# mmbell/Scythe.jl

Hardware: AMD Instinct MI355X
Metric: model steps/sec, RLZ 512x256x64 shallow-water (higher is better)
Workload: dtype f64; 1 GPU; RLZ 513x256x64 (rings x azimuth x levels), 6 vars, 7 derivative slots, Oneway_ShallowWater_HeightResolvedBL, uniform ring table kmax<=127, b_zDim 43; num_cells=171, tiles=1, exchange=none, exchange_impl=none, device_busy_before_warmup=500 steps of the timed model, nan=False

## Files before the change

### include/scythe_hip.h

```cpp
#ifndef SCYTHE_HIP_H
#define SCYTHE_HIP_H

#include <stddef.h>
#include <stdint.h>

#ifdef __cplusplus
extern "C" {
#endif

#define SX_ABI_VERSION 2

enum { SX_GEOM_R = 0, SX_GEOM_RZ = 1, SX_GEOM_RL = 2, SX_GEOM_RLZ = 3 };

enum { SX_BC_R0 = 0, SX_BC_R1T0 = 1, SX_BC_R1T1 = 2, SX_BC_R1T2 = 3, SX_BC_R2T10 = 4, SX_BC_R2T20 = 5, SX_BC_R3 = 6,
       SX_BC_PERIODIC = 7 };

enum {
    SX_EQ_LINEAR_ADVECTION_1D = 0,
    SX_EQ_LINEAR_ADVECTION_RZ = 1,
    SX_EQ_LINEAR_ADVECTION_RL = 2,
    SX_EQ_LINEAR_ADVECTION_RLZ = 3,
    SX_EQ_ONEWAY_SW_SLAB = 4,
    SX_EQ_TWOWAY_SW_SLAB = 5,
    SX_EQ_ONEWAY_SW_HRBL = 6,
// ... 61 lines not shown
int sx_abi_version(void);
int sx_equation_set_id(const char *name);
int sx_get_dims(const sx_handle *h, sx_dims *out);
int sx_set_stream(sx_handle *h, void *hip_stream);
int sx_synchronize(sx_handle *h);

int sx_get_gridpoints(const sx_handle *h, double *out);
int sx_calc_tile_sizes(const sx_grid_desc *patch, int32_t n_tiles, double *out);

int sx_cheb_column_ops(double zmin, double zmax, int32_t zDim, int32_t b_zDim, int32_t bcb, int32_t bct, double *z,
                       double *rec, double *dz, double *dzz, double *integ);

int sx_spline_solve_check(int32_t num_cells, double xmin, double xmax, double l_q, int32_t bcl, int32_t bcr, const double *b,
                          double *a_pcr, double *a_chol, int32_t *levels);

enum { SX_PLAN_FORWARD = 0, SX_PLAN_ZINV = 1, SX_PLAN_PCR = 2 };
int sx_launch_plan(int32_t kind, const int32_t *in, int32_t *out, char *kernel, int32_t kernel_cap);

int sx_set_physical_values(sx_handle *h, const double *values);
int sx_get_physical(sx_handle *h, double *out);
int sx_get_var_np1(sx_handle *h, double *out);
int sx_get_tile_spectral(sx_handle *h, double *out);
int sx_set_patch_spectral_b(sx_handle *h, const double *shared);
int sx_get_patch_spectral_a(sx_handle *h, double *out);
int sx_set_patch_spectral_a(sx_handle *h, const double *a);

int sx_index_map_sizes(const sx_handle *h, int64_t *n_owned, int64_t *n_halo);
int sx_index_maps(const sx_handle *h, int64_t *patch_owned, int64_t *tile_owned, int64_t *patch_halo, int64_t *tile_halo);

int sx_state_size(const sx_handle *h, int64_t *n_doubles);
int sx_get_state(sx_handle *h, double *out);
// ... 51 lines not shown
```

### scythe.jl_amd/csrc/sx_api.cpp

```cpp
#include "sx_internal.hpp"
#include <algorithm>
#include <array>
#include <cmath>
#include <cstdlib>
#include <cstring>
#include <map>
#include <type_traits>

namespace sx {

static thread_local std::string g_err;
static thread_local bool g_err_set = false;

void set_error(const std::string &msg) {
    if (!g_err_set) g_err = msg;
    g_err_set = true;
}
void clear_error() { g_err_set = false; }
static int status() { return g_err_set ? 1 : 0; }
int error_status() { return status(); }

#define HIPOK(x)                                                                          \
    do {                                                                                  \
        hipError_t e_ = (x);                                                              \
// ... 626 lines not shown
                    j.mat_off = ((int64_t)v * 3 + sz) * h->nz * h->Zb;
                    jf.push_back(j);
                    const int need = sz == 0 ? horiz : sz == 1 ? z : zz;
                    if (eq[v] & need) je.push_back(j);
                }
                ColJob f;
                f.in_off = (int64_t)v * h->nz * h->K2;
                f.out_off = (int64_t)v * h->Zb * h->K2;
                f.mat_off = 0;
                jz.push_back(f);
            }
            h->njobs_zinv_full = (int)jf.size();
            h->njobs_zinv_eq = (int)je.size();
            if (!upload(h, &h->d_jobs_zinv_full, jf) || !upload(h, &h->d_jobs_zinv_eq, je) || !upload(h, &h->d_jobs_zf, jz)) FAIL();
        }
    }
    {
        std::vector<int64_t> ao(h->b_rDim), neg(h->b_rDim, -1);
        for (int m = 0; m < h->b_rDim; m++) ao[m] = (int64_t)m * h->C;
        if (hipMemcpy(h->d_aoff, ao.data(), sizeof(int64_t) * ao.size(), hipMemcpyHostToDevice) != hipSuccess ||
            hipMemcpy(h->d_neg1, neg.data(), sizeof(int64_t) * neg.size(), hipMemcpyHostToDevice) != hipSuccess) {
            set_error("hipMemcpy H2D failed");
            FAIL();
        }
    }
    h->v_lo = 0; h->v_cnt = h->V;
    h->defer_diag = h->sw.defer_diag && h->eq == SX_EQ_ONEWAY_SW_HRBL && h->V == 6 && h->ncells == h->nc && mfma_shape(h, true) &&
                    h->sw.sbw_mfma;
    if (sx_bind_patch_b(h, nullptr, nullptr)) FAIL();
    *out = h;
// ... 7 lines not shown
#ifdef SX_PHASES
    phases_dump();
    fft_phases_dump();
    sbw_phases_dump();
    dft_phases_dump();
#endif
    graphs_release(h);
    if (h->graph_stream) hipStreamDestroy(h->graph_stream);
    comm_release(h);
    iface_release(h);
    pcr_release(h);
    for (auto &p : h->pending) { hipEventDestroy(p.a); hipEventDestroy(p.b); }
    for (auto e : h->event_pool) hipEventDestroy(e);
    if (h->ev_fork) hipEventDestroy(h->ev_fork);
    if (h->ev_join) hipEventDestroy(h->ev_join);
    if (h->stream2) hipStreamDestroy(h->stream2);
    for (void *p : h->allocs) hipFree(p);
    delete h;
    return 0;
}

int sx_cheb_column_ops(double zmin, double zmax, int32_t zDim, int32_t b_zDim, int32_t bcb, int32_t bct, double *z,
                       double *rec, double *dz, double *dzz, double *integ) {
    clear_error();
    if (zDim < 2 || !(zmax > zmin)) { set_error("sx_cheb_column_ops: need zDim >= 2 and zmax > zmin"); return 1; }
    const int Zb = b_zDim > 0 ? std::min(b_zDim, zDim) : std::min(zDim, (2 * zDim - 1) / 3 + 1);
    ChebOps o;
    std::string err;
    if (!build_cheb_ops(zmin, zmax, zDim, Zb, bcb, bct, o, err)) { set_error(err); return 1; }
    const size_t n2 = (size_t)zDim * zDim;
// ... 14 lines not shown
    std::string err;
    const int nb = num_cells + 3;
    if (!build_spline_class(num_cells, (xmax - xmin) / num_cells, l_q > 0 ? l_q : 2.0, bcl, bcr, sc, err) || !build_pcr_tables(sc, nb, t, err)) {
        set_error(err);
        return 1;
    }
    if (a_pcr) pcr_apply_host(t, nb, b, a_pcr);
    if (a_chol) cholesky_apply_host(sc, nb, b, a_chol);
    if (levels) *levels = t.levels;
    return 0;
}

int sx_launch_plan(int32_t kind, const int32_t *in, int32_t *out, char *kernel, int32_t kernel_cap) {
    clear_error();
    if (!in || !out) { set_error("sx_launch_plan: null argument"); return 1; }
    if (kind != SX_PLAN_FORWARD && kind != SX_PLAN_ZINV && kind != SX_PLAN_PCR) { set_error("sx_launch_plan: unknown kind " + std::to_string(kind)); return 1; }
    const int first = kind == SX_PLAN_PCR ? 0 : 1, last = kind == SX_PLAN_FORWARD ? 6 : kind == SX_PLAN_ZINV ? 3 : 4;
    for (int i = first; i < last; i++)
        if (in[i] < 1) { set_error("sx_launch_plan: dimensions must be positive"); return 1; }
    const Switches sw = read_switches();
    std::string name;
    if (kind == SX_PLAN_FORWARD) {
        const SbPlan p = plan_sb(in[0], in[1], in[2], in[3], in[4], in[5], in[6], sw);
        name = kernel_name(p.kernel);
        const int32_t o[6] = {p.threads, p.bw, p.groups, p.nseg, p.cps, p.segs};
        std::copy(o, o + 6, out);
    } else if (kind == SX_PLAN_ZINV) {
        const ZinvPlan p = plan_zinv(in[0], in[1], in[2], in[3], sw);
        name = kernel_name(p);
        out[0] = p.CT; out[1] = p.grid_x;
// ... 237 lines not shown
}

}

namespace sx {
void flush_diag(sx_handle *h) {
    if (!h->diag_dirty) return;
    h->diag_dirty = false;
    h->v_lo = h->V - 1; h->v_cnt = 1;
    launch_fl_forward(h);
    launch_sb(h);
    launch_solve(h);
    h->v_lo = 0; h->v_cnt = h->V;
}

static void step_launches(sx_handle *h, int t, bool solve) {
    launch_zinv(h, false);
    launch_inverse_and_physics(h, t);
    if (h->defer_diag) { h->v_cnt = h->V - 1; h->diag_dirty = true; }
    launch_fl_forward(h);
    launch_sb(h);
    if (solve) launch_solve(h);
    h->v_cnt = h->V;
}
}

extern "C" {

int sx_spectral_transform(sx_handle *h) {
    clear_error();
    if (!h) { set_error("null handle"); return 1; }
    h->diag_dirty = false;
    launch_fl_forward(h);
    launch_sb(h);
    return status();
}

// ... 343 lines not shown
```

### scythe.jl_amd/csrc/sx_fft.hip

```cpp
#include "sx_internal.hpp"
#include <cstdlib>
#include <cstdio>
#include <vector>

namespace sx {

template <int LOGL, int HL = 0> struct FftCfg {
    static constexpr int FZC = 16, FNP = FZC / 2, LOGZ = 4, SKEW = (LOGL <= 8) ? 2 : 0;
    static constexpr int L4 = (1 << LOGL) / 4;
    static constexpr int LPT = (L4 > 64 ? 64 : L4) >> HL;
    static constexpr int NB = L4 / LPT;
    static constexpr int NK = 2 * NB;
};

#ifdef SX_PHASES
__device__ long long *g_fft_dbg = nullptr;
#define FFT_STAMP(i) do { if (NODE && threadIdx.x == 0 && g_fft_dbg) g_fft_dbg[((int64_t)(blockIdx.z * gridDim.y + blockIdx.y) * gridDim.x + blockIdx.x) * 8 + (i)] = (long long)__builtin_readcyclecounter(); } while (0)
#else
#define FFT_STAMP(i) do { } while (0)
#endif

__device__ __forceinline__ double2 cmul(double2 a, double2 b) { return make_double2(a.x * b.x - a.y * b.y, a.x * b.y + a.y * b.x); }
__device__ __forceinline__ double2 cadd(double2 a, double2 b) { return make_double2(a.x + b.x, a.y + b.y); }
__device__ __forceinline__ double2 csub(double2 a, double2 b) { return make_double2(a.x - b.x, a.y - b.y); }
// ... 558 lines not shown
}

static int fft_fzc(int) { return 16; }
static size_t fft_lds(int L, int sets = 1, bool reg = false) { return sizeof(double2) * ((size_t)sets * (fft_fzc(L) / 2) * (L + (reg ? L / 16 + 2 : L <= 256 ? 2 : 0)) + (reg ? (L == 512 ? 448 : 192) : 0)); }
static int fft_threads(int L, int hl = 0) { return std::max(64, (fft_fzc(L) / 2) * (std::min(L / 4, 64) >> hl)); }

struct InvTarget {
    double *out;
    const double *phi;
    const int *kmax;
    const int64_t *pstart, *phoff;
    int n_units, n_phi;
    int64_t N;
    int node_mode;
    int unit0 = 0;
};

template <int LOGL>
static void launch_inv(sx_handle *h, const int *d_mask, const InvTarget &tg, const double *az, int64_t azrow) {
    const int L = 1 << LOGL;
    dim3 g((h->nz + fft_fzc(L) - 1) / fft_fzc(L), tg.n_units, h->V);
#define INV_LAUNCH_V(NODE, ST, AT, HL, SETS)                                                                                         \
    do {                                                                                                                             \
        if (fft_lds(L, SETS) > 65536)                                                                                                \
            HIPCHK(hipFuncSetAttribute(reinterpret_cast<const void *>(k_rl_inverse_fft<LOGL, 1, NODE, ST, AT, HL, SETS>),           \
                                        hipFuncAttributeMaxDynamicSharedMemorySize, (int)fft_lds(L, SETS)));                        \
        hipLaunchKernelGGL((k_rl_inverse_fft<LOGL, 1, NODE, ST, AT, HL, SETS>), g, dim3(fft_threads(L, HL)), fft_lds(L, SETS), h->stream, \
                           reinterpret_cast<const AT *>(az), planes_of<ST>(tg.out, h->V, tg.N), tg.phi, tg.kmax, tg.pstart,          \
                           h->d_tw, tg.phoff, h->d_ph, d_mask, h->V, h->nz, h->nsz, h->K2, tg.n_phi, tg.N, azrow, h->slot[0],        \
                           h->slot[1], h->slot[2], h->slot[3], h->slot[4], h->slot[5], h->slot[6], nullptr, (int64_t)0, nullptr, 0,  \
                           tg.unit0);                                                                                                \
    } while (0)
#define INV_LAUNCH_REG(NODE, ST, AT)                                                                                                 \
    do {                                                                                                                             \
        constexpr int RS = 2;                                                                                                        \
        if (fft_lds(L, RS, true) > 65536)                                                                                            \
// ... 41 lines not shown
}

template <int LOGL>
static void launch_fwd(sx_handle *h, dim3 g) {
    const int L = 1 << LOGL;
    if (h->sp32)
        hipLaunchKernelGGL((k_fl_forward_fft<LOGL, float>), g, dim3(fft_threads(L)), fft_lds(L), h->stream, h->d_np1 + (int64_t)h->v_lo * h->N,
                           reinterpret_cast<float *>(h->d_Fl) + (int64_t)h->v_lo * h->nz * h->K2,
                           h->d_kmax, h->d_pstart, h->d_tw, h->d_phoff, h->d_ph, h->V, h->nz, h->K2, h->N);
    else
        hipLaunchKernelGGL((k_fl_forward_fft<LOGL, double>), g, dim3(fft_threads(L)), fft_lds(L), h->stream, h->d_np1 + (int64_t)h->v_lo * h->N,
                           h->d_Fl + (int64_t)h->v_lo * h->nz * h->K2, h->d_kmax,
                           h->d_pstart, h->d_tw, h->d_phoff, h->d_ph, h->V, h->nz, h->K2, h->N);
}

void launch_rl_inverse_fft(sx_handle *h, const int *d_mask, int n_rings) {
    const int id = timer_id(h, "k_rl_inverse");
    timer_begin(h, id);
    InvTarget tg{h->d_phys, h->d_phi, h->d_kmax, h->d_pstart, h->d_phoff, n_rings < 0 ? h->nrings : n_rings, h->nrings, h->N, 0};
    launch_inv_any(h, d_mask, tg);
    timer_end(h);
}

#ifdef SX_PHASES
static long long *g_fft_buf = nullptr;
static int64_t g_fft_n = 0;
void fft_phases_dump() {
    const char *path = getenv("SX_FFT_PHASES_OUT");
    if (!path || !g_fft_buf) return;
    std::vector<long long> hst((size_t)g_fft_n * 8);
    hipDeviceSynchronize();
    hipMemcpy(hst.data(), g_fft_buf, sizeof(long long) * hst.size(), hipMemcpyDeviceToHost);
    FILE *f = fopen(path, "wb");
    if (f) { fwrite(hst.data(), sizeof(long long), hst.size(), f); fclose(f); }
}
#endif

void launch_node_fft(sx_handle *h) {
    const int id = timer_id(h, "k_node_fft");
    timer_begin(h, id);
#ifdef SX_PHASES
    if (!g_fft_buf) {
        g_fft_n = (int64_t)((h->nz + fft_fzc(h->uniform_L) - 1) / fft_fzc(h->uniform_L)) * h->V * h->nbt;
        hipMalloc(&g_fft_buf, sizeof(long long) * g_fft_n * 8);
        hipMemset(g_fft_buf, 0, sizeof(long long) * g_fft_n * 8);
        hipMemcpyToSymbol(HIP_SYMBOL(g_fft_dbg), &g_fft_buf, sizeof(g_fft_buf));
    }
#endif
    const int j0 = h->R_in / MUBAR;
    InvTarget tg{h->d_G, h->d_nphi, h->d_nkmax, h->d_npstart, h->d_nphoff, h->nbt - j0, h->nbt, h->NG, 1, j0};
    launch_inv_any(h, h->d_mask_node, tg);
    timer_end(h);
}

void launch_fl_forward_fft(sx_handle *h) {
    const int id = timer_id(h, "k_fl_forward");
    timer_begin(h, id);
    const int fzc = fft_fzc(h->uniform_L);
    dim3 g((h->nz + fzc - 1) / fzc, h->v_cnt, h->nrings);
    switch (ilog2(h->uniform_L)) {
        case 4: launch_fwd<4>(h, g); break;
        case 5: launch_fwd<5>(h, g); break;
        case 6: launch_fwd<6>(h, g); break;
        case 7: launch_fwd<7>(h, g); break;
        case 8: launch_fwd<8>(h, g); break;
        default: launch_fwd<9>(h, g); break;
// ... 7 lines not shown
```

### scythe.jl_amd/csrc/sx_internal.hpp

```cpp
#pragma once
#include <hip/hip_runtime.h>
#include <cmath>
#include <cstdint>
#include <string>
#include <utility>
#include <vector>
#include "scythe_hip.h"

#define HIPCHK(x)                                                                                   \
    do {                                                                                            \
        hipError_t e_ = (x);                                                                        \
        if (e_ != hipSuccess) ::sx::set_error(std::string(#x) + ": " + hipGetErrorString(e_) + " (" __FILE__ ":" + std::to_string(__LINE__) + ")"); \
    } while (0)

namespace sx {

void set_error(const std::string &msg);

constexpr int DFT_KMAX_SINGLE = 319;
constexpr int MUBAR = 3;

struct SplineClass {
    int bcl = 0, bcr = 0;
    int nfree = 0, periodic = 0, rl = 0, rr = 0;
// ... 112 lines not shown
    SbKernel kernel = SbKernel::refused;
    int threads = 0, bw = 0;
    int groups = 0, nseg = 0, cps = 0, segs = 0;
};
enum class ZinvKernel { none , colmat, mfma_2_1, mfma_4_1, mfma_4_2, mfma_8_1, mfma_8_2, mfma_8_4 };
struct ZinvPlan {
    ZinvKernel kernel = ZinvKernel::none;
    bool f32 = false;
    int CT = 1, grid_x = 0;
};
struct PcrPlan { int R = 1, logR = 0, threads = 64; };
constexpr int PCR_IPT = 4;
SbPlan plan_sb(int geometry, int nz, int Zb, int K2, int v_cnt, int ncells, int sp32, const Switches &sw);
ZinvPlan plan_zinv(int geometry, int nz, int K2, int sp32, const Switches &sw);
PcrPlan plan_pcr(int nblk_max, int b_rDim, int K2, int ngroups, const Switches &sw);
std::string kernel_name(SbKernel k);
std::string kernel_name(const ZinvPlan &p);

struct Timer {
    const char *name;
    double ms = 0.0;
    int64_t calls = 0;
};

struct PendingEvent {
    int timer;
    hipEvent_t a, b;
};

}
// ... 15 lines not shown
    double ts = 0;
    int eq = SX_EQ_NONE, semi = 0, w_index = 0, xi_index = 0, col_var = 0;
    double par[SX_NPARAMS] = {};
    int rot = 0;
    hipStream_t stream = nullptr;
    double *d_A = nullptr, *d_Bfull = nullptr, *d_Btile = nullptr, *d_Btile_own = nullptr;
    const double *d_Bsrc = nullptr;
    int64_t *d_rowoff = nullptr, *d_aoff = nullptr, *d_neg1 = nullptr;
    int a2a_n = 0, a2a_me = 0, a2a_g0 = 0, a2a_g1 = 0;
    std::vector<int64_t> a2a_colstart;
    std::vector<int> a2a_cell0, a2a_ncells;
    int *d_a2a_owner = nullptr;
    int64_t *d_a2a_soff = nullptr, *d_a2a_cw = nullptr, *d_a2a_cs = nullptr, *d_a2a_offA = nullptr, *d_a2a_offB = nullptr;
    hipStream_t stream2 = nullptr;
    hipEvent_t ev_fork = nullptr, ev_join = nullptr;
    int *d_dft_items[3] = {nullptr, nullptr, nullptr};
    int n_dft_items[3] = {0, 0, 0};
    int n_dft_big[3] = {0, 0, 0};
    int dft_lcap_small = 0, dft_kcap_small = 0;
    int plain_steps = 0;
    hipGraphExec_t graph_exec[3] = {nullptr, nullptr, nullptr};
    hipStream_t graph_stream = nullptr;
    int *d_rlq_items[2] = {nullptr, nullptr};
    int n_rlq_items[2] = {0, 0};
    int defer_diag = 0, v_lo = 0, v_cnt = 0;
    bool diag_dirty = false;
    std::vector<int> hmask_full, hmask_eq;
    bool in_advance = false;
    bool L_all_mult4 = false;
    sx::CellConsts cell_consts = {};
// ... 33 lines not shown
    sx::ColJob *d_jobs_zinv_full = nullptr, *d_jobs_zinv_eq = nullptr, *d_jobs_zf = nullptr;
    int njobs_zinv_full = 0, njobs_zinv_eq = 0, last_zinv_jobs = 0, last_zinv_rows = 0;
    int ncls = 0;
    size_t dev_bytes = 0;
    std::vector<void *> allocs;
    int timers_on = 0;
    bool timer_skip = false;
    std::string timer_only;
    std::vector<sx::Timer> timers;
    std::vector<sx::PendingEvent> pending;
    std::vector<hipEvent_t> event_pool;
};

namespace sx {
inline dim3 grid1(int64_t n, int bs) { return dim3((unsigned)((n + bs - 1) / bs)); }
void launch_zinv(sx_handle *h, bool full);
void launch_rl_inverse(sx_handle *h, bool full);
bool fft_path_ok(const sx_handle *h);
inline bool mfma_levels(int nz) { return nz == 32 || nz == 64 || nz == 128; }
inline bool mfma_shape(const sx_handle *h, bool zb_bound = false) {
    return fft_path_ok(h) && h->has_z && mfma_levels(h->nz) && (!zb_bound || (h->nz <= 64 ? h->Zb <= 64 : h->Zb <= 96));
}
bool fft_fused_zinv(const sx_handle *h);
bool dft_mfma_ok(const sx_handle *h);
void launch_rl_inverse_dft(sx_handle *h, const int *d_mask);
void launch_fl_forward_dft(sx_handle *h);
void launch_rl_inverse_fft(sx_handle *h, const int *d_mask, int n_rings = -1);
void launch_node_fft(sx_handle *h);
void launch_fl_forward_fft(sx_handle *h);
void launch_physics(sx_handle *h, int t);
void launch_inverse_and_physics(sx_handle *h, int t);
void launch_copy_slot0(sx_handle *h);
void launch_fl_forward(sx_handle *h);
void launch_sb(sx_handle *h);
void launch_solve(sx_handle *h);
void launch_solve_a2a(sx_handle *h, const double *recv, double *send);
void launch_a2a_pack(sx_handle *h, double *buf, int unpack);
void launch_halo_add(sx_handle *h, const double *recv);
void launch_nan_check(sx_handle *h);
void launch_max_abs(sx_handle *h, unsigned long long *d_out);
int timer_id(sx_handle *h, const char *name);
void timer_begin(sx_handle *h, int id);
void timer_end(sx_handle *h);
void timers_flush(sx_handle *h);
void clear_error();
int error_status();
void comm_release(sx_handle *h);
void flush_diag(sx_handle *h);
void graphs_release(sx_handle *h);
void iface_release(sx_handle *h);
// ... 17 lines not shown
```

### scythe.jl_amd/csrc/sx_kernels.hip

```cpp
#include "sx_internal.hpp"
#include <cmath>

namespace sx {

constexpr int ZC = 16;

__global__ void __launch_bounds__(256)
k_colmat(const double *__restrict__ in, double *__restrict__ out, const double *__restrict__ mats,
         const ColJob *__restrict__ jobs, int n_in, int n_out, int K2, int64_t in_row, int64_t out_row, int row0) {
    extern __shared__ double As[];
    const int lane = threadIdx.x;
    const int g = __builtin_amdgcn_readfirstlane(threadIdx.y);
    const int blk = blockIdx.x * 64 + lane;
    const ColJob job = jobs[blockIdx.y];
    const double *src = in + (int64_t)(row0 + blockIdx.z) * in_row + job.in_off;
    double *dst = out + (int64_t)blockIdx.z * out_row + job.out_off;
    const double *M = mats + job.mat_off;
    const bool ok = blk < K2;
    for (int i = g; i < n_in; i += 4) As[i * 64 + lane] = ok ? src[(int64_t)i * K2 + blk] : 0.0;
    __syncthreads();
    for (int o0 = g * 4; o0 < n_out; o0 += 16) {
        const double *m0 = M + (int64_t)o0 * n_in;
        const double *m1 = M + (int64_t)min(o0 + 1, n_out - 1) * n_in;
        const double *m2 = M + (int64_t)min(o0 + 2, n_out - 1) * n_in;
// ... 735 lines not shown

#ifdef SX_PHASES
static long long *g_sbw_buf = nullptr;
static int64_t g_sbw_n = 0;
void sbw_phases_dump() {
    const char *path = getenv("SX_SBW_PHASES_OUT");
    if (!path || !g_sbw_buf) return;
    std::vector<long long> hst((size_t)g_sbw_n * 8);
    hipDeviceSynchronize();
    hipMemcpy(hst.data(), g_sbw_buf, sizeof(long long) * hst.size(), hipMemcpyDeviceToHost);
    FILE *f = fopen(path, "wb");
    if (f) { fwrite(hst.data(), sizeof(long long), hst.size(), f); fclose(f); }
}
#endif

void launch_zinv(sx_handle *h, bool full) {
    if (!h->has_z || rz_fused(h)) return;
    const int id = timer_id(h, "k_zinv");
    timer_begin(h, id);
    const int njobs = full ? h->njobs_zinv_full : h->njobs_zinv_eq;
    h->last_zinv_jobs = njobs;
    if (njobs > 0) {
        const int rows = (!full && h->node_mode && fft_fused_zinv(h)) ? (h->R_in > 0 ? std::min(h->nbt, h->R_in / MUBAR + 3) : 0) : h->nbt;
        h->last_zinv_rows = rows;
        if (rows == 0) { timer_end(h); return; }
        const ZinvPlan p = plan_zinv(h->geom, h->nz, h->K2, h->sp32, h->sw);
        dim3 g(p.grid_x, njobs, rows);
        const ColJob *jobs = full ? h->d_jobs_zinv_full : h->d_jobs_zinv_eq;
        const int64_t azrow = (int64_t)h->V * 3 * h->nz * h->K2;
#define ZINV_T(MT, OT, CT) hipLaunchKernelGGL((k_colmat_mfma<MT, OT, CT>), g, dim3(256), 0, h->stream, h->d_A, reinterpret_cast<OT *>(h->d_Az), h->d_MzT, jobs, h->Zb, h->K2, h->C, azrow, h->cell0)
#define ZINV(MT, CT) if (p.f32) ZINV_T(MT, float, CT); else ZINV_T(MT, double, CT); break
        switch (p.kernel) {
        case ZinvKernel::mfma_2_1: ZINV(2, 1);
        case ZinvKernel::mfma_4_1: ZINV(4, 1);
        case ZinvKernel::mfma_4_2: ZINV(4, 2);
        case ZinvKernel::mfma_8_1: ZINV(8, 1);
        case ZinvKernel::mfma_8_2: ZINV(8, 2);
        case ZinvKernel::mfma_8_4: ZINV(8, 4);
        case ZinvKernel::colmat:
            hipLaunchKernelGGL(k_colmat, g, dim3(64, 4), sizeof(double) * 64 * h->Zb, h->stream, h->d_A, h->d_Az, h->d_Mz, jobs,
                               h->Zb, h->nz, h->K2, h->C, azrow, h->cell0);
            break;
        case ZinvKernel::none: break;
// ... 46 lines not shown
    const int id = timer_id(h, "k_fl_forward");
    timer_begin(h, id);
    const int xstride = h->L_max | 1;
    const size_t lds = sizeof(double) * ZC * xstride;
    if (lds > 64 * 1024) {
        set_error("azimuthal forward transform: rings of " + std::to_string(h->L_max) + " points are outside every transform path (power-of-two ring tables up to 512 points, ring lengths that are multiples of 4 up to 5120 points, any length up to 511 points)");
        return;
    }
    dim3 g((h->nz + ZC - 1) / ZC, h->V, h->nrings);
    hipLaunchKernelGGL(k_fl_forward, g, dim3(256), lds, h->stream, h->d_np1, h->d_Fl, h->d_L, h->d_kmax, h->d_pstart,
                       h->d_twoff, h->d_tw, h->d_phoff, h->d_ph, h->V, h->nz, h->K2, h->N, h->has_l, xstride);
    HIPCHK(hipGetLastError());
    timer_end(h);
}

void launch_sb(sx_handle *h) {
    const SbPlan p = plan_sb(h->geom, h->nz, h->Zb, h->K2, h->v_cnt, h->ncells, h->sp32, h->sw);
    if (p.kernel == SbKernel::rz_forward) { launch_rz_forward(h); return; }
    if (p.kernel == SbKernel::refused) { set_error("launch_sb: fp32 ring spectra (storage_f32 = 2) need the matrix-core sliding-window kernel"); return; }
    const int id = timer_id(h, h->has_z ? "k_sbz" : "k_sb");
    timer_begin(h, id);
    if (p.kernel == SbKernel::sb) {
        const int64_t plane = (int64_t)h->V * h->nz * h->K2;
        dim3 g((unsigned)((plane + 255) / 256), h->nbt);
        hipLaunchKernelGGL(k_sb, g, dim3(p.threads), 0, h->stream, h->d_Fl, h->d_Btile, h->d_phi, h->d_wq, h->ncells, plane);
    } else if (p.kernel == SbKernel::sbz) {
        dim3 g((h->K2 + p.bw - 1) / p.bw, h->V, h->nbt);
        hipLaunchKernelGGL(k_sbz, g, dim3(64, 4), sizeof(double) * 64 * h->nz, h->stream, h->d_Fl, h->d_Btile, h->d_phi, h->d_wq,
                           h->d_CB, h->ncells, h->V, h->nz, h->Zb, h->K2, h->C);
    } else {
        dim3 gw((h->K2 + p.bw - 1) / p.bw, h->v_cnt, p.segs);
        const int64_t flo = (int64_t)h->v_lo * h->nz * h->K2, blo = (int64_t)h->v_lo * h->Zb * h->K2;
// ... 18 lines not shown
        case SbKernel::mfma_64_t256: SBW(double, k_sbw_mfma<64, 32, 256>);
        case SbKernel::mfma_128: SBW(double, k_sbw_mfma<128, 32>);
        case SbKernel::mfma_32_f32: SBW(float, k_sbw_mfma<32, 64, 512, float>);
        case SbKernel::mfma_64_f32: SBW(float, k_sbw_mfma<64, 64, 512, float>);
        case SbKernel::mfma_64_t256_f32: SBW(float, k_sbw_mfma<64, 32, 256, float>);
        case SbKernel::mfma_128_f32: SBW(float, k_sbw_mfma<128, 32, 512, float>);
        default: break;
        }
#undef SBW
    }
    HIPCHK(hipGetLastError());
    timer_end(h);
}


void launch_solve(sx_handle *h) {
    const int id = timer_id(h, "k_solve");
    timer_begin(h, id);
    dim3 g((h->K2 > 1 ? (h->K2 / 2 - 1 + 63) / 64 : 0) + 1, h->V * h->Zb);
    const bool contiguous = (h->d_Bsrc == h->d_Bfull);
    const int ngroups = contiguous ? h->v_cnt * h->Zb : h->V * h->Zb;
    if (pcr_wanted(h, (int64_t)ngroups * (h->K2 > 1 ? h->K2 - 1 : 1))) {
        const int64_t clo = contiguous ? (int64_t)h->v_lo * h->Zb * h->K2 : 0;
        launch_solve_pcr(h, contiguous, h->d_Bsrc + clo, h->d_rowoff, h->d_neg1, h->d_A + clo, h->d_aoff, h->d_neg1,
                         contiguous ? h->v_lo * h->Zb : 0, ngroups, h->C);
        timer_end(h);
        return;
    }
    if (contiguous) {
        const int64_t clo = (int64_t)h->v_lo * h->Zb * h->K2;
        g.y = h->v_cnt * h->Zb;
        hipLaunchKernelGGL(k_solve<true>, g, dim3(64), sizeof(double) * 4 * h->b_rDim, h->stream, h->d_Bsrc + clo, h->d_rowoff, h->d_neg1, h->d_A + clo, h->d_aoff, h->d_neg1,
                           h->d_cls, h->d_cmeta, h->d_gl, h->d_gr, h->d_Lband, h->d_Ldinv, h->d_Larrow, h->b_rDim, h->Zb, h->K2, h->v_lo * h->Zb,
                           h->C);
    }
    else
        hipLaunchKernelGGL(k_solve<false>, g, dim3(64), sizeof(double) * 8 * h->b_rDim, h->stream, h->d_Bsrc, h->d_rowoff, h->d_neg1, h->d_A, h->d_aoff,
// ... 63 lines not shown
```

### scythe.jl_amd/csrc/sx_physics.hip

```cpp
#include "sx_internal.hpp"

namespace sx {

template <class ST>
struct PhysArgsT {
    Planes<ST> P;
    double *En;
    double *E1, *E2;
    double *In;
    double *np1;
    const double *r, *cosl, *sinl, *z;
    const double *MintT, *MdzT;
    int64_t N;
    int V, nz, t, eq;
    int s_u, s_r, s_rr, s_l, s_ll, s_z, s_zz;
    double ts;
    double par[SX_NPARAMS];
    int64_t col0, col1;
    Planes<ST> G;
    const double *phi;
    const double *ref;
    int write_w;
    int64_t NG;
    int L, nrings;
// ... 1098 lines not shown
        const size_t lds = sizeof(int) * 2 * cpb * (1 + h->nz);
        hipLaunchKernelGGL(k_condensation, grid1(h->Nh, cpb), dim3(cpb * h->nz), lds, h->stream, h->d_np1, h->d_ref, h->N, h->nz, cpb);
        HIPCHK(hipGetLastError());
        timer_end(h);
    }
    if (h->eq != SX_EQ_NONE && part != 1) h->rot = (h->rot + 2) % 3;
}

static void launch_physics_part(sx_handle *h, int t, int part) {
    if (h->f32) launch_physics_t<float>(h, t, part);
    else launch_physics_t<double>(h, t, part);
}

void launch_physics(sx_handle *h, int t) { launch_physics_part(h, t, 0); }

void launch_inverse_and_physics(sx_handle *h, int t) {
    struct Scope { sx_handle *h; Scope(sx_handle *x) : h(x) { h->in_advance = true; } ~Scope() { h->in_advance = false; } } scope(h);
    const bool two = h->node_mode && h->R_in > 0 && h->sw.overlap && h->eq == SX_EQ_ONEWAY_SW_HRBL && !h->semi;
    if (!two) {
        launch_rl_inverse(h, false);
        launch_physics(h, t);
        return;
    }
    h->last_mask_full = false;
    h->node_active = 1;
    if (!h->stream2) {
        HIPCHK(hipStreamCreateWithFlags(&h->stream2, hipStreamNonBlocking));
        HIPCHK(hipEventCreateWithFlags(&h->ev_fork, hipEventDisableTiming));
        HIPCHK(hipEventCreateWithFlags(&h->ev_join, hipEventDisableTiming));
    }
    hipStream_t s0 = h->stream;
    HIPCHK(hipEventRecord(h->ev_fork, s0));
    HIPCHK(hipStreamWaitEvent(h->stream2, h->ev_fork, 0));
    h->stream = h->stream2;
    launch_rl_inverse_fft(h, h->d_mask_eq, h->R_in);
    launch_physics_part(h, t, 1);
    HIPCHK(hipEventRecord(h->ev_join, h->stream2));
    h->stream = s0;
    launch_node_fft(h);
    if (h->sw.overlap == 2) HIPCHK(hipStreamWaitEvent(s0, h->ev_join, 0));
    launch_physics_part(h, t, 2);
    if (h->sw.overlap != 2) HIPCHK(hipStreamWaitEvent(s0, h->ev_join, 0));
}

}
```

### scythe.jl_amd/csrc/sx_plan.cpp

```cpp
#include "sx_internal.hpp"
#include <algorithm>

namespace sx {

static bool fused_rz(int geometry, int sp32, const Switches &sw) { return sw.rz_fused && geometry == SX_GEOM_RZ && !sp32; }

SbPlan plan_sb(int geometry, int nz, int Zb, int K2, int v_cnt, int ncells, int sp32, const Switches &sw) {
    SbPlan p;
    if (fused_rz(geometry, sp32, sw)) { p.kernel = SbKernel::rz_forward; return p; }
    if (geometry != SX_GEOM_RZ && geometry != SX_GEOM_RLZ) { p.kernel = SbKernel::sb; p.threads = 256; return p; }
    if (nz != 32 && nz != 64 && nz != 128) { p.kernel = SbKernel::sbz; p.threads = 256; p.bw = 64; return p; }
    const bool mf = sw.sbw_mfma && (nz <= 64 ? Zb <= 64 : Zb <= 96);
    if (sp32 && !mf) return p;
    const bool t256 = sw.sbw_t256 && mf && nz == 64;
    const bool narrow = (mf && nz == 128) || t256;
    const bool pf = (sw.sbw_prefetch && nz <= 64) || mf;
    p.threads = t256 ? 256 : 512;
    p.bw = narrow ? 32 : 64;
    p.groups = ((K2 + p.bw - 1) / p.bw) * v_cnt;
    p.nseg = sw.sbw_seg > 0 ? sw.sbw_seg : std::max(1, (narrow ? 512 : pf || nz == 128 ? 256 : 384) / p.groups);
    p.cps = std::max(ncells <= 64 ? 2 : 6, (ncells + p.nseg - 1) / p.nseg);
    p.segs = (ncells + p.cps - 1) / p.cps;
    using K = SbKernel;
    if (sp32) p.kernel = t256 ? K::mfma_64_t256_f32 : nz == 64 ? K::mfma_64_f32 : nz == 32 ? K::mfma_32_f32 : K::mfma_128_f32;
// ... 15 lines not shown
               : nz == 128 ? (p.CT == 1 ? K::mfma_8_1 : p.CT == 4 ? K::mfma_8_4 : K::mfma_8_2) : K::colmat;
    return p;
}

PcrPlan plan_pcr(int nblk_max, int b_rDim, int K2, int ngroups, const Switches &sw) {
    PcrPlan p;
    const int64_t total = (int64_t)ngroups * (K2 > 1 ? K2 - 1 : 1);
    int R = sw.pcr_r > 0 ? sw.pcr_r : total <= 4096 ? 4 : total <= 16384 ? 8 : 16;
    while (R > 1 && (int64_t)nblk_max * R > 1024) R >>= 1;
    while ((1 << (p.logR + 1)) <= R) p.logR++;
    p.R = 1 << p.logR;
    p.threads = std::min(1024, ((std::max(nblk_max * p.R, (b_rDim * p.R + PCR_IPT - 1) / PCR_IPT) + 63) / 64) * 64);
    return p;
}

std::string kernel_name(SbKernel k) {
    static const char *const NAMES[] = {
        "", "k_sb", "k_sbz", "k_rz_forward", "k_sbw<32, false>", "k_sbw<32, true>", "k_sbw<64, false>", "k_sbw<64, true>", "k_sbw<128, false>",
        "k_sbw_mfma<32>", "k_sbw_mfma<64>", "k_sbw_mfma<64, 32, 256>", "k_sbw_mfma<128, 32>", "k_sbw_mfma<32, 64, 512, float>",
        "k_sbw_mfma<64, 64, 512, float>", "k_sbw_mfma<64, 32, 256, float>", "k_sbw_mfma<128, 32, 512, float>"};
    static_assert(sizeof(NAMES) / sizeof(NAMES[0]) == (size_t)SbKernel::mfma_128_f32 + 1, "one name per SbKernel");
    return NAMES[(int)k];
}

std::string kernel_name(const ZinvPlan &p) {
    if (p.kernel == ZinvKernel::none) return "";
    if (p.kernel == ZinvKernel::colmat) return "k_colmat";
    static const int MT[] = {2, 4, 4, 8, 8, 8};
    return "k_colmat_mfma<" + std::to_string(MT[(int)p.kernel - (int)ZinvKernel::mfma_2_1]) + ", " + (p.f32 ? "float" : "double") + ", " +
           std::to_string(p.CT) + ">";
// ... 4 lines not shown
```

Before: 1020 steps/s.

## Pipeline inverse and forward stages across two streams by variable groups

Splits the variables into two cost-balanced groups and runs zinv, node FFT, ring inverse, forward FFT, sliding-window and solve stages for each group on two HIP streams linked by events. The second group trails the first so their kernels can overlap and fill the GPU better. This adds extra launches, event waits and per-group job and mask tables, and only applies in the overlap==1 HRBL node mode without timers or graphs. Smaller per-group launches may use the device less efficiently.

```diff
diff --git a/include/scythe_hip.h b/include/scythe_hip.h
--- a/include/scythe_hip.h
+++ b/include/scythe_hip.h
@@ -99,7 +99,7 @@
 int sx_spline_solve_check(int32_t num_cells, double xmin, double xmax, double l_q, int32_t bcl, int32_t bcr, const double *b,
                           double *a_pcr, double *a_chol, int32_t *levels);
 
-enum { SX_PLAN_FORWARD = 0, SX_PLAN_ZINV = 1, SX_PLAN_PCR = 2 };
+enum { SX_PLAN_FORWARD = 0, SX_PLAN_ZINV = 1, SX_PLAN_PCR = 2, SX_PLAN_GROUPS = 3 };
 int sx_launch_plan(int32_t kind, const int32_t *in, int32_t *out, char *kernel, int32_t kernel_cap);
 
 int sx_set_physical_values(sx_handle *h, const double *values);
diff --git a/profiles/trace_overlap.py b/profiles/trace_overlap.py
--- /dev/null
+++ b/profiles/trace_overlap.py
@@ -0,0 +1,37 @@
+#!/usr/bin/env python3
+import csv
+import re
+import sys
+from collections import defaultdict
+
+
+def short(name):
+    m = re.match(r"(?:void )?(?:sx::)?(\w+)", name)
+    return m.group(1) if m else name
+
+
+def main():
+    rows = []
+    with open(sys.argv[1], newline="") as f:
+        for r in csv.DictReader(f):
+            rows.append((int(r["Start_Timestamp"]), int(r["End_Timestamp"]), short(r["Kernel_Name"])))
+    rows.sort()
+    rows = rows[-(int(sys.argv[2]) if len(sys.argv) > 2 else 4000):]
+    pair, alone, open_ = defaultdict(int), defaultdict(int), []
+    for s, e, n in rows:
+        open_ = [(oe, on) for oe, on in open_ if oe > s]
+        for oe, on in open_:
+            if on != n:
+                pair[tuple(sorted((on, n)))] += min(oe, e) - s
+        open_.append((e, n))
+        alone[n] += e - s
+    span = rows[-1][1] - rows[0][0]
+    busy = sum(alone.values())
+    print("%d dispatches over %.3f ms; kernel time summed %.3f ms (%.3f x the span)" % (len(rows), span / 1e6, busy / 1e6, busy / span))
+    print("%-44s %12s %10s" % ("pair of different kernels in flight together", "overlap ms", "of span"))
+    for k, v in sorted(pair.items(), key=lambda kv: -kv[1]):
+        print("%-44s %12.3f %9.1f%%" % (" + ".join(k), v / 1e6, 100.0 * v / span))
+
+
+if __name__ == "__main__":
+    main()
diff --git a/scythe.jl_amd/csrc/sx_api.cpp b/scythe.jl_amd/csrc/sx_api.cpp
--- a/scythe.jl_amd/csrc/sx_api.cpp
+++ b/scythe.jl_amd/csrc/sx_api.cpp
@@ -664,6 +664,33 @@
             h->njobs_zinv_eq = (int)je.size();
             if (!upload(h, &h->d_jobs_zinv_full, jf) || !upload(h, &h->d_jobs_zinv_eq, je) || !upload(h, &h->d_jobs_zf, jz)) FAIL();
         }
+        if (h->node_mode && h->has_z) {
+            std::vector<int> cost(h->V);
+            for (int v = 0; v < h->V; v++) cost[v] = __builtin_popcount(eq[v]);
+            h->inv_groups = plan_var_groups(cost.data(), h->V);
+            for (int k = 0; k < 2 && h->inv_groups.n == 2; k++) {
+                const int lo = h->inv_groups.lo[k], hi = lo + h->inv_groups.cnt[k];
+                std::vector<int> me(h->V, 0), mn(h->V, 0);
+                std::vector<ColJob> jg;
+                const int horiz = u | r | rr | l | ll;
+                for (int v = lo; v < hi; v++) {
+                    me[v] = eq[v];
+                    if (eq[v] & (u | r | rr)) mn[v] |= u;
+                    mn[v] |= eq[v] & (l | ll | z | zz);
+                    for (int sz = 0; sz < 3; sz++) {
+                        if (!(eq[v] & (sz == 0 ? horiz : sz == 1 ? z : zz))) continue;
+                        ColJob j;
+                        j.in_off = (int64_t)v * h->Zb * h->K2;
+                        j.out_off = ((int64_t)v * 3 + sz) * h->nz * h->K2;
+                        j.mat_off = ((int64_t)v * 3 + sz) * h->nz * h->Zb;
+                        jg.push_back(j);
+                    }
+                }
+                h->njobs_zinv_grp[k] = (int)jg.size();
+                if (jg.empty()) jg.push_back(ColJob{0, 0, 0});
+                if (!upload(h, &h->d_jobs_zinv_grp[k], jg) || !upload(h, &h->d_mask_eq_grp[k], me) || !upload(h, &h->d_mask_node_grp[k], mn)) FAIL();
+            }
+        }
     }
     {
         std::vector<int64_t> ao(h->b_rDim), neg(h->b_rDim, -1);
@@ -701,6 +728,7 @@
     for (auto e : h->event_pool) hipEventDestroy(e);
     if (h->ev_fork) hipEventDestroy(h->ev_fork);
     if (h->ev_join) hipEventDestroy(h->ev_join);
+    for (auto e : h->ev_pipe) if (e) hipEventDestroy(e);
     if (h->stream2) hipStreamDestroy(h->stream2);
     for (void *p : h->allocs) hipFree(p);
     delete h;
@@ -745,6 +773,14 @@
 int sx_launch_plan(int32_t kind, const int32_t *in, int32_t *out, char *kernel, int32_t kernel_cap) {
     clear_error();
     if (!in || !out) { set_error("sx_launch_plan: null argument"); return 1; }
+    if (kind == SX_PLAN_GROUPS) {
+        if (in[0] < 0) { set_error("sx_launch_plan: a negative number of variables"); return 1; }
+        const VarGroups g = plan_var_groups(in + 1, in[0]);
+        const int32_t o[5] = {g.n, g.lo[0], g.cnt[0], g.lo[1], g.cnt[1]};
+        std::copy(o, o + 5, out);
+        if (kernel && kernel_cap > 0) kernel[0] = 0;
+        return 0;
+    }
     if (kind != SX_PLAN_FORWARD && kind != SX_PLAN_ZINV && kind != SX_PLAN_PCR) { set_error("sx_launch_plan: unknown kind " + std::to_string(kind)); return 1; }
     const int first = kind == SX_PLAN_PCR ? 0 : 1, last = kind == SX_PLAN_FORWARD ? 6 : kind == SX_PLAN_ZINV ? 3 : 4;
     for (int i = first; i < last; i++)
@@ -1012,13 +1048,49 @@
     h->v_lo = 0; h->v_cnt = h->V;
 }
 
+static void forward_pipelined(sx_handle *h, bool solve) {
+    const int lo = h->v_lo, cnt = h->v_cnt;
+    const int unit[6] = {1, 1, 1, 1, 1, 1};
+    const VarGroups g = plan_var_groups(unit, cnt);
+    const int64_t cols = (int64_t)cnt * h->Zb * (h->K2 > 1 ? h->K2 - 1 : 1);
+    const bool split_solve = solve && h->d_Bsrc == h->d_Bfull && !pcr_wanted(h, cols);
+    if (g.n < 2) {
+        launch_fl_forward(h);
+        launch_sb(h);
+        if (solve) launch_solve(h);
+        return;
+    }
+    hipStream_t s0 = h->stream, s2 = h->stream2;
+    auto stage = [&](int ev, auto launch) {
+        h->v_lo = lo + g.lo[0]; h->v_cnt = g.cnt[0];
+        launch();
+        HIPCHK(hipEventRecord(h->ev_pipe[ev], s0));
+        HIPCHK(hipStreamWaitEvent(s2, h->ev_pipe[ev], 0));
+        h->v_lo = lo + g.lo[1]; h->v_cnt = g.cnt[1];
+        h->stream = s2;
+        launch();
+        h->stream = s0;
+    };
+    stage(sx_handle::EV_FL, [&] { launch_fl_forward(h); });
+    stage(sx_handle::EV_SB, [&] { launch_sb(h, cnt); });
+    if (split_solve) stage(sx_handle::EV_SOLVE, [&] { launch_solve(h, false); });
+    HIPCHK(hipEventRecord(h->ev_pipe[sx_handle::EV_DONE], s2));
+    HIPCHK(hipStreamWaitEvent(s0, h->ev_pipe[sx_handle::EV_DONE], 0));
+    h->v_lo = lo; h->v_cnt = cnt;
+    if (solve && !split_solve) launch_solve(h);
+}
+
 static void step_launches(sx_handle *h, int t, bool solve) {
-    launch_zinv(h, false);
+    const bool pipe = pipelined(h);
+    if (!pipe) launch_zinv(h, false);
     launch_inverse_and_physics(h, t);
     if (h->defer_diag) { h->v_cnt = h->V - 1; h->diag_dirty = true; }
-    launch_fl_forward(h);
-    launch_sb(h);
-    if (solve) launch_solve(h);
+    if (pipe) forward_pipelined(h, solve);
+    else {
+        launch_fl_forward(h);
+        launch_sb(h);
+        if (solve) launch_solve(h);
+    }
     h->v_cnt = h->V;
 }
 }
diff --git a/scythe.jl_amd/csrc/sx_fft.hip b/scythe.jl_amd/csrc/sx_fft.hip
--- a/scythe.jl_amd/csrc/sx_fft.hip
+++ b/scythe.jl_amd/csrc/sx_fft.hip
@@ -596,12 +596,13 @@
     int64_t N;
     int node_mode;
     int unit0 = 0;
+    int n_vars = 0;
 };
 
 template <int LOGL>
 static void launch_inv(sx_handle *h, const int *d_mask, const InvTarget &tg, const double *az, int64_t azrow) {
     const int L = 1 << LOGL;
-    dim3 g((h->nz + fft_fzc(L) - 1) / fft_fzc(L), tg.n_units, h->V);
+    dim3 g((h->nz + fft_fzc(L) - 1) / fft_fzc(L), tg.n_units, tg.n_vars > 0 ? tg.n_vars : h->V);
 #define INV_LAUNCH_V(NODE, ST, AT, HL, SETS)                                                                                         \
     do {                                                                                                                             \
         if (fft_lds(L, SETS) > 65536)                                                                                                \
@@ -673,10 +674,11 @@
                            h->d_pstart, h->d_tw, h->d_phoff, h->d_ph, h->V, h->nz, h->K2, h->N);
 }
 
-void launch_rl_inverse_fft(sx_handle *h, const int *d_mask, int n_rings) {
+void launch_rl_inverse_fft(sx_handle *h, const int *d_mask, int n_rings, int grp) {
     const int id = timer_id(h, "k_rl_inverse");
     timer_begin(h, id);
-    InvTarget tg{h->d_phys, h->d_phi, h->d_kmax, h->d_pstart, h->d_phoff, n_rings < 0 ? h->nrings : n_rings, h->nrings, h->N, 0};
+    InvTarget tg{h->d_phys, h->d_phi, h->d_kmax, h->d_pstart, h->d_phoff, n_rings < 0 ? h->nrings : n_rings, h->nrings, h->N, 0, 0,
+                 grp >= 0 ? h->inv_groups.cnt[grp] : 0};
     launch_inv_any(h, d_mask, tg);
     timer_end(h);
 }
@@ -695,7 +697,7 @@
 }
 #endif
 
-void launch_node_fft(sx_handle *h) {
+void launch_node_fft(sx_handle *h, int grp) {
     const int id = timer_id(h, "k_node_fft");
     timer_begin(h, id);
 #ifdef SX_PHASES
@@ -707,8 +709,9 @@
     }
 #endif
     const int j0 = h->R_in / MUBAR;
-    InvTarget tg{h->d_G, h->d_nphi, h->d_nkmax, h->d_npstart, h->d_nphoff, h->nbt - j0, h->nbt, h->NG, 1, j0};
-    launch_inv_any(h, h->d_mask_node, tg);
+    InvTarget tg{h->d_G, h->d_nphi, h->d_nkmax, h->d_npstart, h->d_nphoff, h->nbt - j0, h->nbt, h->NG, 1, j0,
+                 grp >= 0 ? h->inv_groups.cnt[grp] : 0};
+    launch_inv_any(h, grp >= 0 ? h->d_mask_node_grp[grp] : h->d_mask_node, tg);
     timer_end(h);
 }
 
diff --git a/scythe.jl_amd/csrc/sx_internal.hpp b/scythe.jl_amd/csrc/sx_internal.hpp
--- a/scythe.jl_amd/csrc/sx_internal.hpp
+++ b/scythe.jl_amd/csrc/sx_internal.hpp
@@ -150,6 +150,8 @@
 SbPlan plan_sb(int geometry, int nz, int Zb, int K2, int v_cnt, int ncells, int sp32, const Switches &sw);
 ZinvPlan plan_zinv(int geometry, int nz, int K2, int sp32, const Switches &sw);
 PcrPlan plan_pcr(int nblk_max, int b_rDim, int K2, int ngroups, const Switches &sw);
+struct VarGroups { int n = 1, lo[2] = {0, 0}, cnt[2] = {0, 0}; };
+VarGroups plan_var_groups(const int *cost, int v_cnt);
 std::string kernel_name(SbKernel k);
 std::string kernel_name(const ZinvPlan &p);
 
@@ -195,6 +197,12 @@
     int64_t *d_a2a_soff = nullptr, *d_a2a_cw = nullptr, *d_a2a_cs = nullptr, *d_a2a_offA = nullptr, *d_a2a_offB = nullptr;
     hipStream_t stream2 = nullptr;
     hipEvent_t ev_fork = nullptr, ev_join = nullptr;
+    enum { EV_ZINV, EV_INV, EV_NODE, EV_FL, EV_SB, EV_SOLVE, EV_DONE, N_EV_PIPE };
+    hipEvent_t ev_pipe[N_EV_PIPE] = {};
+    sx::VarGroups inv_groups;
+    sx::ColJob *d_jobs_zinv_grp[2] = {nullptr, nullptr};
+    int njobs_zinv_grp[2] = {0, 0};
+    int *d_mask_eq_grp[2] = {nullptr, nullptr}, *d_mask_node_grp[2] = {nullptr, nullptr};
     int *d_dft_items[3] = {nullptr, nullptr, nullptr};
     int n_dft_items[3] = {0, 0, 0};
     int n_dft_big[3] = {0, 0, 0};
@@ -258,7 +266,7 @@
 
 namespace sx {
 inline dim3 grid1(int64_t n, int bs) { return dim3((unsigned)((n + bs - 1) / bs)); }
-void launch_zinv(sx_handle *h, bool full);
+void launch_zinv(sx_handle *h, bool full, int grp = -1);
 void launch_rl_inverse(sx_handle *h, bool full);
 bool fft_path_ok(const sx_handle *h);
 inline bool mfma_levels(int nz) { return nz == 32 || nz == 64 || nz == 128; }
@@ -269,15 +277,17 @@
 bool dft_mfma_ok(const sx_handle *h);
 void launch_rl_inverse_dft(sx_handle *h, const int *d_mask);
 void launch_fl_forward_dft(sx_handle *h);
-void launch_rl_inverse_fft(sx_handle *h, const int *d_mask, int n_rings = -1);
-void launch_node_fft(sx_handle *h);
+void launch_rl_inverse_fft(sx_handle *h, const int *d_mask, int n_rings = -1, int grp = -1);
+void launch_node_fft(sx_handle *h, int grp = -1);
 void launch_fl_forward_fft(sx_handle *h);
 void launch_physics(sx_handle *h, int t);
 void launch_inverse_and_physics(sx_handle *h, int t);
 void launch_copy_slot0(sx_handle *h);
 void launch_fl_forward(sx_handle *h);
-void launch_sb(sx_handle *h);
-void launch_solve(sx_handle *h);
+void launch_sb(sx_handle *h, int plan_v = 0);
+void launch_solve(sx_handle *h, bool by_count = true);
+bool pipelined(const sx_handle *h);
+void second_stream(sx_handle *h);
 void launch_solve_a2a(sx_handle *h, const double *recv, double *send);
 void launch_a2a_pack(sx_handle *h, double *buf, int unpack);
 void launch_halo_add(sx_handle *h, const double *recv);
diff --git a/scythe.jl_amd/csrc/sx_kernels.hip b/scythe.jl_amd/csrc/sx_kernels.hip
--- a/scythe.jl_amd/csrc/sx_kernels.hip
+++ b/scythe.jl_amd/csrc/sx_kernels.hip
@@ -773,19 +773,19 @@
 }
 #endif
 
-void launch_zinv(sx_handle *h, bool full) {
+void launch_zinv(sx_handle *h, bool full, int grp) {
     if (!h->has_z || rz_fused(h)) return;
     const int id = timer_id(h, "k_zinv");
     timer_begin(h, id);
-    const int njobs = full ? h->njobs_zinv_full : h->njobs_zinv_eq;
-    h->last_zinv_jobs = njobs;
+    h->last_zinv_jobs = full ? h->njobs_zinv_full : h->njobs_zinv_eq;
+    const int njobs = grp >= 0 ? h->njobs_zinv_grp[grp] : h->last_zinv_jobs;
     if (njobs > 0) {
         const int rows = (!full && h->node_mode && fft_fused_zinv(h)) ? (h->R_in > 0 ? std::min(h->nbt, h->R_in / MUBAR + 3) : 0) : h->nbt;
         h->last_zinv_rows = rows;
         if (rows == 0) { timer_end(h); return; }
         const ZinvPlan p = plan_zinv(h->geom, h->nz, h->K2, h->sp32, h->sw);
         dim3 g(p.grid_x, njobs, rows);
-        const ColJob *jobs = full ? h->d_jobs_zinv_full : h->d_jobs_zinv_eq;
+        const ColJob *jobs = grp >= 0 ? h->d_jobs_zinv_grp[grp] : full ? h->d_jobs_zinv_full : h->d_jobs_zinv_eq;
         const int64_t azrow = (int64_t)h->V * 3 * h->nz * h->K2;
 #define ZINV_T(MT, OT, CT) hipLaunchKernelGGL((k_colmat_mfma<MT, OT, CT>), g, dim3(256), 0, h->stream, h->d_A, reinterpret_cast<OT *>(h->d_Az), h->d_MzT, jobs, h->Zb, h->K2, h->C, azrow, h->cell0)
 #define ZINV(MT, CT) if (p.f32) ZINV_T(MT, float, CT); else ZINV_T(MT, double, CT); break
@@ -862,8 +862,8 @@
     timer_end(h);
 }
 
-void launch_sb(sx_handle *h) {
-    const SbPlan p = plan_sb(h->geom, h->nz, h->Zb, h->K2, h->v_cnt, h->ncells, h->sp32, h->sw);
+void launch_sb(sx_handle *h, int plan_v) {
+    const SbPlan p = plan_sb(h->geom, h->nz, h->Zb, h->K2, plan_v > 0 ? plan_v : h->v_cnt, h->ncells, h->sp32, h->sw);
     if (p.kernel == SbKernel::rz_forward) { launch_rz_forward(h); return; }
     if (p.kernel == SbKernel::refused) { set_error("launch_sb: fp32 ring spectra (storage_f32 = 2) need the matrix-core sliding-window kernel"); return; }
     const int id = timer_id(h, h->has_z ? "k_sbz" : "k_sb");
@@ -912,13 +912,13 @@
 }
 
 
-void launch_solve(sx_handle *h) {
+void launch_solve(sx_handle *h, bool by_count) {
     const int id = timer_id(h, "k_solve");
     timer_begin(h, id);
     dim3 g((h->K2 > 1 ? (h->K2 / 2 - 1 + 63) / 64 : 0) + 1, h->V * h->Zb);
     const bool contiguous = (h->d_Bsrc == h->d_Bfull);
     const int ngroups = contiguous ? h->v_cnt * h->Zb : h->V * h->Zb;
-    if (pcr_wanted(h, (int64_t)ngroups * (h->K2 > 1 ? h->K2 - 1 : 1))) {
+    if (by_count && pcr_wanted(h, (int64_t)ngroups * (h->K2 > 1 ? h->K2 - 1 : 1))) {
         const int64_t clo = contiguous ? (int64_t)h->v_lo * h->Zb * h->K2 : 0;
         launch_solve_pcr(h, contiguous, h->d_Bsrc + clo, h->d_rowoff, h->d_neg1, h->d_A + clo, h->d_aoff, h->d_neg1,
                          contiguous ? h->v_lo * h->Zb : 0, ngroups, h->C);
diff --git a/scythe.jl_amd/csrc/sx_physics.hip b/scythe.jl_amd/csrc/sx_physics.hip
--- a/scythe.jl_amd/csrc/sx_physics.hip
+++ b/scythe.jl_amd/csrc/sx_physics.hip
@@ -1136,30 +1136,57 @@
 
 void launch_physics(sx_handle *h, int t) { launch_physics_part(h, t, 0); }
 
+static bool two_streams(const sx_handle *h) {
+    return h->node_mode && h->R_in > 0 && h->sw.overlap && h->eq == SX_EQ_ONEWAY_SW_HRBL && !h->semi;
+}
+
+bool pipelined(const sx_handle *h) {
+    return two_streams(h) && h->sw.overlap == 1 && !h->timers_on && !h->sw.use_graph && h->has_z && h->inv_groups.n == 2;
+}
+
+void second_stream(sx_handle *h) {
+    if (h->stream2) return;
+    HIPCHK(hipStreamCreateWithFlags(&h->stream2, hipStreamNonBlocking));
+    HIPCHK(hipEventCreateWithFlags(&h->ev_fork, hipEventDisableTiming));
+    HIPCHK(hipEventCreateWithFlags(&h->ev_join, hipEventDisableTiming));
+    for (auto &e : h->ev_pipe) HIPCHK(hipEventCreateWithFlags(&e, hipEventDisableTiming));
+}
+
 void launch_inverse_and_physics(sx_handle *h, int t) {
     struct Scope { sx_handle *h; Scope(sx_handle *x) : h(x) { h->in_advance = true; } ~Scope() { h->in_advance = false; } } scope(h);
-    const bool two = h->node_mode && h->R_in > 0 && h->sw.overlap && h->eq == SX_EQ_ONEWAY_SW_HRBL && !h->semi;
-    if (!two) {
+    if (!two_streams(h)) {
         launch_rl_inverse(h, false);
         launch_physics(h, t);
         return;
     }
+    const bool pipe = pipelined(h);
     h->last_mask_full = false;
     h->node_active = 1;
-    if (!h->stream2) {
-        HIPCHK(hipStreamCreateWithFlags(&h->stream2, hipStreamNonBlocking));
-        HIPCHK(hipEventCreateWithFlags(&h->ev_fork, hipEventDisableTiming));
-        HIPCHK(hipEventCreateWithFlags(&h->ev_join, hipEventDisableTiming));
-    }
-    hipStream_t s0 = h->stream;
+    second_stream(h);
+    hipStream_t s0 = h->stream, s2 = h->stream2;
     HIPCHK(hipEventRecord(h->ev_fork, s0));
-    HIPCHK(hipStreamWaitEvent(h->stream2, h->ev_fork, 0));
-    h->stream = h->stream2;
-    launch_rl_inverse_fft(h, h->d_mask_eq, h->R_in);
+    HIPCHK(hipStreamWaitEvent(s2, h->ev_fork, 0));
+    if (pipe) {
+        launch_zinv(h, false, 0);
+        HIPCHK(hipEventRecord(h->ev_pipe[sx_handle::EV_ZINV], s0));
+        launch_node_fft(h, 0);
+        launch_rl_inverse_fft(h, h->d_mask_eq_grp[0], h->R_in, 0);
+        HIPCHK(hipEventRecord(h->ev_pipe[sx_handle::EV_INV], s0));
+    }
+    h->stream = s2;
+    if (pipe) {
+        HIPCHK(hipStreamWaitEvent(s2, h->ev_pipe[sx_handle::EV_ZINV], 0));
+        launch_zinv(h, false, 1);
+        HIPCHK(hipStreamWaitEvent(s2, h->ev_pipe[sx_handle::EV_INV], 0));
+        launch_node_fft(h, 1);
+        HIPCHK(hipEventRecord(h->ev_pipe[sx_handle::EV_NODE], s2));
+        launch_rl_inverse_fft(h, h->d_mask_eq_grp[1], h->R_in, 1);
+    } else launch_rl_inverse_fft(h, h->d_mask_eq, h->R_in);
     launch_physics_part(h, t, 1);
-    HIPCHK(hipEventRecord(h->ev_join, h->stream2));
+    HIPCHK(hipEventRecord(h->ev_join, s2));
     h->stream = s0;
-    launch_node_fft(h);
+    if (pipe) HIPCHK(hipStreamWaitEvent(s0, h->ev_pipe[sx_handle::EV_NODE], 0));
+    else launch_node_fft(h);
     if (h->sw.overlap == 2) HIPCHK(hipStreamWaitEvent(s0, h->ev_join, 0));
     launch_physics_part(h, t, 2);
     if (h->sw.overlap != 2) HIPCHK(hipStreamWaitEvent(s0, h->ev_join, 0));
diff --git a/scythe.jl_amd/csrc/sx_plan.cpp b/scythe.jl_amd/csrc/sx_plan.cpp
--- a/scythe.jl_amd/csrc/sx_plan.cpp
+++ b/scythe.jl_amd/csrc/sx_plan.cpp
@@ -53,6 +53,24 @@
     return p;
 }
 
+VarGroups plan_var_groups(const int *cost, int v_cnt) {
+    VarGroups g;
+    g.cnt[0] = std::max(v_cnt, 0);
+    if (v_cnt < 2) return g;
+    int64_t total = 0, pre = 0, best = -1;
+    for (int v = 0; v < v_cnt; v++) total += cost[v];
+    int split = 1;
+    for (int s = 1; s < v_cnt; s++) {
+        pre += cost[s - 1];
+        const int64_t d = pre > total - pre ? 2 * pre - total : total - 2 * pre;
+        if (best < 0 || d < best) { best = d; split = s; }
+    }
+    g.n = 2;
+    g.cnt[0] = split;
+    g.lo[1] = split; g.cnt[1] = v_cnt - split;
+    return g;
+}
+
 std::string kernel_name(SbKernel k) {
     static const char *const NAMES[] = {
         "", "k_sb", "k_sbz", "k_rz_forward", "k_sbw<32, false>", "k_sbw<32, true>", "k_sbw<64, false>", "k_sbw<64, true>", "k_sbw<128, false>",
```

After: 938.6 steps/s. -8.0%, worse.
